# nanoporetech/bonito

Hardware: AMD Instinct MI355X
Metric: signal samples/sec/GPU (chunk=10000, batch=512) + read accuracy vs ref (higher is better)
Workload: dtype f16

## Files before the change

### bonito_amd/csrc/beam.hip

```cpp
#include <stdlib.h>

#include "common.h"
#include "kernels.h"
#include <cstring>
#include "../../include/bh_lse_table.h"

namespace bh {

__device__ const float g_lse_tab[BH_LSE_TABLE_SIZE] = {BH_LSE_TABLE_VALUES};

__device__ __forceinline__ float lse2_tab(float a, float b, const float* tab) {
    float m = fmaxf(a, b);
    float d = fabsf(a - b);
    if (!(d < BH_LSE_RANGE)) return m;
    float x = d * BH_LSE_SCALE;
    int i = (int)x;
    float f = x - (float)i;
    float t0 = tab[i];
    float sp = __fmaf_rn(f, tab[i + 1] - t0, t0);
    return m + sp;
}

__device__ __forceinline__ float lse2_tab_nb(float a, float b, const float* tab) {
    const float m = fmaxf(a, b);
// ... 421 lines not shown
            }
        }
#pragma unroll
        for (int i = 0; i < 3; ++i) selm[i] = __ballot(hi[i] || selb[i]);
    }
    int before = 0;
#pragma unroll
    for (int i = 0; i < 3; ++i) {
        sel[i] = (selm[i] >> lane) & 1ull;
        slot[i] = before + popc64(selm[i] & lanemask_lt(lane));
        before += popc64(selm[i]);
    }
    return before;
}

constexpr int NBK = 256;
constexpr int BKE = 2;
constexpr unsigned TAG_MASK = 0x1ffffu;

struct BeamTable {
    int* cnt;
    uint2_t* ent;
    int* ov_cnt;
    uint2_t* ov;
};

__device__ __forceinline__ unsigned bucket_match(const uint4_t& e0, unsigned hash, unsigned want) {
    unsigned d = 32u;
    d = min(d, e0.x == hash ? e0.y - want : 32u);
    d = min(d, e0.z == hash ? e0.w - want : 32u);
    return d;
}

__device__ __forceinline__ void dma16(const char* g, char* lds) {
    const unsigned l = (unsigned)__builtin_amdgcn_readfirstlane((int)(unsigned)(size_t)(__attribute__((address_space(3))) char*)lds);
    asm volatile("s_mov_b32 m0, %0\n\ts_nop 0\n\tglobal_load_lds_dwordx4 %1, off" ::"s"(l), "v"(g) : "memory");
}
__device__ __forceinline__ void dma16_nt(const char* g, char* lds) {
    const unsigned l = (unsigned)__builtin_amdgcn_readfirstlane((int)(unsigned)(size_t)(__attribute__((address_space(3))) char*)lds);
    asm volatile("s_mov_b32 m0, %0\n\ts_nop 0\n\tglobal_load_lds_dwordx4 %1, off nt" ::"s"(l), "v"(g) : "memory");
}

#include "../../include/bh_bs2.h"
typedef float float2_t __attribute__((ext_vector_type(2)));

__device__ __forceinline__ float2_t fma2(float2_t a, float2_t b, float2_t c) { return __builtin_elementwise_fma(a, b, c); }
__device__ __forceinline__ float2_t splat2(float v) { return float2_t{v, v}; }

__device__ __forceinline__ float2_t bs2_exp2(float2_t x) {
    x.x = __builtin_amdgcn_fmed3f(x.x, -BH_BS2_XMAX, BH_BS2_XMAX);
    x.y = __builtin_amdgcn_fmed3f(x.y, -BH_BS2_XMAX, BH_BS2_XMAX);
    const float2_t t = fma2(x, splat2(BH_BS2_LOG2E), splat2(BH_BS2_MAGIC));
    const float2_t n = t - splat2(BH_BS2_MAGIC);
    const float2_t f = fma2(x, splat2(BH_BS2_LOG2E), -n);
    float2_t p = splat2(BH_BS2_E5);
    p = fma2(p, f, splat2(BH_BS2_E4));
    p = fma2(p, f, splat2(BH_BS2_E3));
    p = fma2(p, f, splat2(BH_BS2_E2));
    p = fma2(p, f, splat2(BH_BS2_E1));
    p = fma2(p, f, splat2(BH_BS2_E0));
    float2_t r;
    r.x = __uint_as_float(__float_as_uint(p.x) + (__float_as_uint(t.x) << 23));
    r.y = __uint_as_float(__float_as_uint(p.y) + (__float_as_uint(t.y) << 23));
    return r;
}
__device__ __forceinline__ float bs2_exp1(float x) { return bs2_exp2(float2_t{x, x}).x; }
// ... 28 lines not shown
        v = fmaxf(v, dpp_f<0x4E, 0xF>(v));
    }
    if constexpr (GL >= 16) {
        v = fmaxf(v, dpp_f<0x124, 0xF>(v));
        v = fmaxf(v, dpp_f<0x128, 0xF>(v));
    }
    if constexpr (GL == 64) {
        v = fmaxf(v, dpp_f<0x142, 0xA>(v));
        v = fmaxf(v, dpp_f<0x143, 0xC>(v));
        v = __builtin_bit_cast(float, __builtin_amdgcn_readlane(__builtin_bit_cast(int, v), 63));
    }
    return v;
}
template <int GL>
__device__ __forceinline__ float group_sum(float v) {
    if constexpr (GL >= 4) {
        v += dpp_f<0xB1, 0xF>(v);
        v += dpp_f<0x4E, 0xF>(v);
    }
    if constexpr (GL >= 16) {
        v += dpp_f<0x124, 0xF>(v);
        v += dpp_f<0x128, 0xF>(v);
    }
    if constexpr (GL == 64) {
        const float r1 = __builtin_bit_cast(float, __builtin_amdgcn_readlane(__builtin_bit_cast(int, v), 15));
        const float r2 = __builtin_bit_cast(float, __builtin_amdgcn_readlane(__builtin_bit_cast(int, v), 31));
        const float r3 = __builtin_bit_cast(float, __builtin_amdgcn_readlane(__builtin_bit_cast(int, v), 47));
        const float r4 = __builtin_bit_cast(float, __builtin_amdgcn_readlane(__builtin_bit_cast(int, v), 63));
        v = (r1 + r2) + (r3 + r4);
    }
    return v;
}

template <int STATE_LEN>
struct Bs2Geo {
    static constexpr int S = 1 << (2 * STATE_LEN), Q = S / 4;
    static constexpr int GL = Q < 64 ? Q : 64;
    static constexpr int CPWV = 64 / GL;
    static constexpr int WPC = Q <= 64 ? 1 : Q / 64;
    static constexpr int UT = WPC * 64;
    static constexpr int UPB = CPWV > 1 ? 1 : 256 / UT;
    static constexpr int CPB = UPB * CPWV;
    static constexpr int ROW = 4 * S * 2;
    static constexpr int PP = CPWV * S / 2;
    static constexpr int UNIT_LDS = 2 * BS2_R * CPWV * ROW + CPWV * 2 * S * 4 + 64;
};

template <int STATE_LEN>
__global__ __launch_bounds__(256) void bs2_backward_kernel(Bs2Args p) {
    using G = Bs2Geo<STATE_LEN>;
    constexpr int S = G::S, Q = G::Q, WPC = G::WPC, GL = G::GL, CPWV = G::CPWV;
    extern __shared__ __attribute__((aligned(16))) char smem[];
    const int T = p.T;
    const int unit = threadIdx.x / G::UT, tu = threadIdx.x - unit * G::UT;
    const int lane = threadIdx.x & 63, wv = tu >> 6;
    const int c = WPC == 1 ? lane / GL : 0;
    const int m = WPC == 1 ? lane - c * GL : tu;
    const int n0 = (blockIdx.x * G::UPB + unit) * CPWV;
    const int n = n0 + c;
    const bool live = n < p.N;
    const int nn = live ? n : p.N - 1;
    char* mine = smem + (size_t)unit * G::UNIT_LDS;
    half_t* rows = (half_t*)mine;
    float* pb = (float*)(mine + 2 * BS2_R * CPWV * G::ROW) + (size_t)c * 2 * S;
    float* mxs = (float*)(mine + 2 * BS2_R * CPWV * G::ROW) + (size_t)CPWV * 2 * S;
    float* bn = p.b + (long)nn * (T + 1) * S;
    const float eb = bs2_exp1(p.blank);

    auto stage = [&](int k) {
        const int u0 = k * BS2_R, nr = min(BS2_R, T - u0);
        for (int r = 0; r < nr; ++r) {
            char* dst = (char*)(rows + (size_t)((k & 1) * BS2_R + r) * CPWV * 4 * S);
            const long trow = (long)(T - 1 - (u0 + r)) * 4 * S;
#pragma unroll
            for (int i0 = 0; i0 < G::PP; i0 += G::UT) {
                const int q = i0 + wv * 64 + lane;
                const int qc = q / (S / 2), qp = q - qc * (S / 2);
                const int qn = min(n0 + qc, p.N - 1);
                const char* src = (const char*)(p.scores + (long)qn * T * 4 * S + trow) + (long)qp * 16;
                if (p.nt) dma16_nt(src, dst + (size_t)(i0 + wv * 64) * 16);
                else dma16(src, dst + (size_t)(i0 + wv * 64) * 16);
            }
        }
    };
#pragma unroll
    for (int l = 0; l < 4; ++l) pb[m + l * Q] = 1.0f;
    if (WPC > 1 && tu < 4) mxs[tu] = 1.0f;
    if (WPC == 1 && live) {
#pragma unroll
        for (int l = 0; l < 4; ++l) bn[(long)T * S + m + l * Q] = 1.0f;
    }
    if (T > 0) stage(0);
    int cur = 0;
    const int nblk = (T + BS2_R - 1) / BS2_R;
    for (int k = 0; k < nblk; ++k) {
        const int u0 = k * BS2_R, nr = min(BS2_R, T - u0);
        asm volatile("s_waitcnt vmcnt(0)" ::: "memory");
        if (WPC > 1) __syncthreads();
        if (k + 1 < nblk) stage(k + 1);
        for (int r = 0; r < nr; ++r) {
            const int t = T - 1 - (u0 + r);
            const float* prev = pb + cur * S;
            const half_t* row = rows + ((size_t)((k & 1) * BS2_R + r) * CPWV + c) * 4 * S;
            const uint4_t w0 = *(const uint4_t*)(row + 16 * m);
            const uint4_t w1 = *(const uint4_t*)(row + 16 * m + 8);
            float4_t succ = *(const float4_t*)(prev + 4 * m);
            float own[4];
#pragma unroll
            for (int l = 0; l < 4; ++l) own[l] = prev[m + l * Q];
            if (WPC > 1) {
                const float4_t mv = *(const float4_t*)(mxs + cur * 4);
                const float mx = fmaxf(fmaxf(mv.x, mv.y), fmaxf(mv.z, mv.w));
                const unsigned eb23 = ((__float_as_uint(mx) >> 23) - 127u) << 23;
#pragma unroll
                for (int l = 0; l < 4; ++l) own[l] = __uint_as_float(__float_as_uint(own[l]) - eb23);
#pragma unroll
                for (int x = 0; x < 4; ++x) succ[x] = __uint_as_float(__float_as_uint(succ[x]) - eb23);
                if (live) {
#pragma unroll
                    for (int l = 0; l < 4; ++l) {
                        if (p.nt) __builtin_nontemporal_store(own[l], bn + (long)(t + 1) * S + m + l * Q);
                        else bn[(long)(t + 1) * S + m + l * Q] = own[l];
                    }
                }
            }
            const unsigned w[8] = {w0.x, w0.y, w0.z, w0.w, w1.x, w1.y, w1.z, w1.w};
            float2_t acc01, acc23;
            acc01 = fma2(splat2(eb), float2_t{own[0], own[1]}, splat2(BH_BS2_TINY));
            acc23 = fma2(splat2(eb), float2_t{own[2], own[3]}, splat2(BH_BS2_TINY));
#pragma unroll
            for (int x = 0; x < 4; ++x) {
                const half2_t h01 = __builtin_bit_cast(half2_t, w[2 * x]), h23 = __builtin_bit_cast(half2_t, w[2 * x + 1]);
                const float2_t e01 = bs2_exp2(float2_t{(float)h01.x, (float)h01.y});
                const float2_t e23 = bs2_exp2(float2_t{(float)h23.x, (float)h23.y});
                acc01 = fma2(e01, splat2(succ[x]), acc01);
                acc23 = fma2(e23, splat2(succ[x]), acc23);
// ... 3 lines not shown
            float* nextb = pb + (cur ^ 1) * S;
            if (WPC > 1) {
                if (lane == 0) mxs[(cur ^ 1) * 4 + wv] = mx;
#pragma unroll
                for (int l = 0; l < 4; ++l) nextb[m + l * Q] = raw[l];
                __syncthreads();
            } else {
                const unsigned eb23 = ((__float_as_uint(mx) >> 23) - 127u) << 23;
#pragma unroll
                for (int l = 0; l < 4; ++l) raw[l] = __uint_as_float(__float_as_uint(raw[l]) - eb23);
#pragma unroll
                for (int l = 0; l < 4; ++l) nextb[m + l * Q] = raw[l];
                if (live) {
#pragma unroll
                    for (int l = 0; l < 4; ++l) {
                        if (p.nt) __builtin_nontemporal_store(raw[l], bn + (long)t * S + m + l * Q);
                        else bn[(long)t * S + m + l * Q] = raw[l];
                    }
                }
            }
            cur ^= 1;
        }
    }
    if (WPC > 1 && live) {
        const float* prev = pb + cur * S;
        const float4_t mv = *(const float4_t*)(mxs + cur * 4);
        const float mx = fmaxf(fmaxf(mv.x, mv.y), fmaxf(mv.z, mv.w));
        const unsigned eb23 = ((__float_as_uint(mx) >> 23) - 127u) << 23;
#pragma unroll
        for (int l = 0; l < 4; ++l) bn[m + l * Q] = __uint_as_float(__float_as_uint(prev[m + l * Q]) - eb23);
    }
}

template <int STATE_LEN>
__host__ __device__ constexpr int beam_wave_lds() {
    constexpr int S = 1 << (2 * STATE_LEN), BTB = beam_btb<STATE_LEN>();
    return 2 * (BTB * 4 * S * 2 + BTB * S * 4) + NBK * BKE * 8 + MAXW * (16 + 8 + 8) + (NBK + 4) * 4 + BTB * MAXW;
}
constexpr int BEAM_TAB_LDS = (BH_LSE_TABLE_SIZE + 2) * 4;

template <int STATE_LEN>
__host__ __device__ constexpr int scan_wave_lds() { return 2 * (1 << (2 * STATE_LEN)) * 4 + 64; }
__device__ __forceinline__ float wave_sum_f32(float v) {
    v += dpp_f<0xB1, 0xF>(v);
    v += dpp_f<0x4E, 0xF>(v);
    v += dpp_f<0x124, 0xF>(v);
    v += dpp_f<0x128, 0xF>(v);
    const float r1 = __builtin_bit_cast(float, __builtin_amdgcn_readlane(__builtin_bit_cast(int, v), 15));
    const float r2 = __builtin_bit_cast(float, __builtin_amdgcn_readlane(__builtin_bit_cast(int, v), 31));
    const float r3 = __builtin_bit_cast(float, __builtin_amdgcn_readlane(__builtin_bit_cast(int, v), 47));
    const float r4 = __builtin_bit_cast(float, __builtin_amdgcn_readlane(__builtin_bit_cast(int, v), 63));
    return (r1 + r2) + (r3 + r4);
}

template <int STATE_LEN>
__device__ __forceinline__ void scan_lin_lane(float ebl, const half_t* row, const float* ap, int m, float (&anew)[4]) {
    constexpr int S = 1 << (2 * STATE_LEN), Q = S / 4;
    const uint4_t w0 = *(const uint4_t*)(row + 16 * m), w1 = *(const uint4_t*)(row + 16 * m + 8);
    const float4_t own = *(const float4_t*)(ap + 4 * m);
    float pr[4];
#pragma unroll
    for (int r = 0; r < 4; ++r) pr[r] = ap[r * Q + m];
    const unsigned w[8] = {w0.x, w0.y, w0.z, w0.w, w1.x, w1.y, w1.z, w1.w};
#pragma unroll
    for (int k = 0; k < 4; ++k) {
        const half2_t cap = {(half_t)BH_BS2_XMAX, (half_t)BH_BS2_XMAX};
        const half2_t h01 = __builtin_elementwise_min(__builtin_bit_cast(half2_t, w[2 * k]), cap);
        const half2_t h23 = __builtin_elementwise_min(__builtin_bit_cast(half2_t, w[2 * k + 1]), cap);
        float a = __fmaf_rn(ebl, own[k], BH_BS2_TINY);
        a = __fmaf_rn(__expf((float)h01.x), pr[0], a);
        a = __fmaf_rn(__expf((float)h01.y), pr[1], a);
        a = __fmaf_rn(__expf((float)h23.x), pr[2], a);
        a = __fmaf_rn(__expf((float)h23.y), pr[3], a);
        anew[k] = a;
    }
}

template <int STATE_LEN>
__device__ __forceinline__ void scan_step(float ebl, const half_t* row, const float* bnext, float* ap, float* an, int m, bool act, float* Pt) {
    constexpr int S = 1 << (2 * STATE_LEN), Q = S / 4, GL = Q < 64 ? Q : 64;
    float anew[4];
    scan_lin_lane<STATE_LEN>(ebl, row, ap, m, anew);
    const float4_t bnext4 = *(const float4_t*)(bnext + 4 * m);
    const float mx = group_max<GL>(fmaxf(fmaxf(anew[0], anew[1]), fmaxf(anew[2], anew[3])));
    const unsigned e23 = ((__float_as_uint(mx) >> 23) - 127u) << 23;
    float4_t o;
#pragma unroll
    for (int k = 0; k < 4; ++k) o[k] = __uint_as_float(__float_as_uint(anew[k]) - e23);
    if (act) *(float4_t*)(an + 4 * m) = o;
    float cls[4];
#pragma unroll
    for (int k = 0; k < 4; ++k) cls[k] = group_sum<GL>(o[k] * bnext4[k]);
    const float inv = 1.0f / ((cls[0] + cls[1]) + (cls[2] + cls[3]));
    if (GL == 1) {
        if (act) *(float4_t*)Pt = float4_t{cls[0] * inv, cls[1] * inv, cls[2] * inv, cls[3] * inv};
    } else if (act && m < 4) {
        Pt[m] = (m == 0 ? cls[0] : m == 1 ? cls[1] : m == 2 ? cls[2] : cls[3]) * inv;
    }
}

struct Bs2FwdArgs {
    const half_t* scores;
    const float* b;
    float* P;
    int N, T;
    float blank;
// ... 132 lines not shown
    char* mine = smem + BEAM_TAB_LDS + wave * beam_wave_lds<STATE_LEN>();
    half_t* st_sc = (half_t*)mine;
    float* st_b = (float*)(st_sc + 2 * BTB * 4 * S);
    constexpr int SCAN_LDS = scan_wave_lds<STATE_LEN>();
    char* scan_mem = smem + BEAM_TAB_LDS + CPW * beam_wave_lds<STATE_LEN>() + wave * SCAN_LDS;
    if (scan_role) {
        float* al = (float*)scan_mem;
        const int sm = QS >= 64 ? lane : lane - (lane / GLS) * GLS;
        if (slot_ok) *(float4_t*)(al + 4 * sm) = float4_t{1.0f, 1.0f, 1.0f, 1.0f};
        const float ebl = __expf(__builtin_amdgcn_fmed3f(p.blank, -BH_BS2_XMAX, BH_BS2_XMAX));
        float* Pn = p.P + (long)n * T * 4;
        int cb = 0;
        for (int tb0 = 0, blk = 0; tb0 < T; tb0 += BTB, ++blk) {
            const int nsteps = min(BTB, T - tb0);
            __syncthreads();
            const half_t* blk_sc = st_sc + (blk & 1) * BTB * 4 * S;
            const float* blk_b = st_b + (blk & 1) * BTB * S;
            for (int u = 0; u < nsteps; ++u) {
                scan_step<STATE_LEN>(ebl, blk_sc + u * 4 * S, blk_b + u * S, al + cb * S, al + (cb ^ 1) * S, sm, slot_ok, Pn + (long)(tb0 + u) * 4);
                cb ^= 1;
            }
        }
        return;
    }
    BeamTable tb;
    tb.ent = (uint2_t*)(st_b + 2 * BTB * S);
    uint4_t* b_elem = (uint4_t*)(tb.ent + NBK * BKE);
    uint2_t* m_pair = (uint2_t*)(b_elem + MAXW);
    tb.ov = m_pair + MAXW;
    tb.cnt = (int*)(tb.ov + MAXW);
    tb.ov_cnt = tb.cnt + NBK;
    int* hist = tb.cnt;
    uint8_t* st_bp = (uint8_t*)(tb.ov_cnt + 4);

    const half_t* sc = p.scores + (long)n * T * 4 * S;
    const float* bn = p.beta + (long)n * (T + 1) * S;
    uint8_t* bpn = p.bp + (long)n * T * MAXW;

    long long dsec[6] = {0, 0, 0, 0, 0, 0};
    const int ce[3] = {lane & (MAXW - 1), lane >> 2, 16 + (lane >> 2)};
    const int mx = lane & 3;
    const bool stay_lane = lane < MAXW;

    int nb;
#pragma unroll
    for (int i = 0; i < NBK * BKE / 64; ++i) tb.ent[lane + 64 * i] = uint2_t{0u, 0xffffffffu};
    if (lane < MAXW) tb.ov[lane] = uint2_t{0u, 0xffffffffu};
    *(uint4_t*)(tb.cnt + 4 * lane) = uint4_t{0u, 0u, 0u, 0u};
    if (lane < 4) tb.ov_cnt[lane] = 0;
    if (lane < MAXW) m_pair[lane] = uint2_t{0u, 0xffffffffu};
    if (lane < MAXW) b_elem[lane] = uint4_t{0u, 0u, 0u, 0u};
    {
        const int per = (S + 63) / 64;
        unsigned prefix = 0u;
        const int want = W < S ? W : S;
        for (int bit = 31; bit >= 0; --bit) {
            const unsigned trial = prefix | (1u << bit);
            int cnt = 0;
            for (int i = 0; i < per; ++i) {
                const int s = i * 64 + lane;
                const unsigned u = s < S ? bs_ukey(bn[s]) : 0u;
                cnt += popc64(__ballot(u >= trial));
            }
            if (cnt >= want) prefix = trial;
        }
        int n_gt = 0;
        for (int i = 0; i < per; ++i) {
            const int s = i * 64 + lane;
            const unsigned u = s < S ? bs_ukey(bn[s]) : 0u;
            n_gt += popc64(__ballot(u > prefix));
        }
        const int need = want - n_gt;
// ... 25 lines not shown
        dma_rows((const char*)(bn + (long)(tb0 + 1) * S), (char*)(st_b + which * BTB * S), nsteps * S / 4);
    };
    if (T > 0) stage(0, 0);
    for (int tb0 = 0, blk = 0; tb0 < T; tb0 += BTB, ++blk) {
        const int nsteps = min(BTB, T - tb0);
        {
            long long ts0 = 0;
            if (DBG) ts0 = __builtin_readcyclecounter();
            asm volatile("s_waitcnt vmcnt(0)" ::: "memory");
            if (FUSE) __syncthreads();
            if (DBG) dsec[5] += __builtin_readcyclecounter() - ts0;
            if (tb0 + BTB < T) stage(tb0 + BTB, (blk + 1) & 1);
        }
        const half_t* blk_sc = st_sc + (blk & 1) * BTB * 4 * S;
        const float* blk_b = st_b + (blk & 1) * BTB * S;
        for (int u = 0; u < nsteps; ++u) {
            const half_t* row = blk_sc + u * 4 * S;
            const float* b1 = blk_b + u * S;
            const unsigned tag = ((unsigned)(tb0 + u) & TAG_MASK) << 15;
            long long tc0 = 0;
            if (DBG) tc0 = __builtin_readcyclecounter();
            float cs[3];
            unsigned ch[3];
            int cst[3], cinfo[3];
            uint4_t el[3];
#pragma unroll
            for (int i = 0; i < 3; ++i) el[i] = b_elem[ce[i]];
            float mv[3], bg[3];
            uint4_t ent0[3];
            {
                const int es = (int)(el[0].x & (unsigned)(S - 1));
                cst[0] = es; ch[0] = el[0].y; cinfo[0] = ce[0];
                bg[0] = b1[es];
                if (stay_lane && ce[0] < nb) {
                    const int bk = (int)(ch[0] & (NBK - 1));
                    const int pos = atomicAdd(&tb.cnt[bk], 1);
                    const uint2_t e{ch[0], tag | ((unsigned)es << 5) | (unsigned)lane};
                    if (pos < BKE) tb.ent[bk * BKE + pos] = e;
                    else tb.ov[atomicAdd(tb.ov_cnt, 1)] = e;
                }
            }
#pragma unroll
            for (int i = 1; i < 3; ++i) {
                const int es = (int)(el[i].x & (unsigned)(S - 1));
                const int s2 = ((es << 2) | mx) & (S - 1);
                cst[i] = s2;
                ch[i] = bs_mix(el[i].y, mx);
                cinfo[i] = ce[i] | (1 << 5) | (mx << 6);
                mv[i] = (float)row[s2 * 4 + (es >> sh)];
                bg[i] = b1[s2];
                ent0[i] = *(const uint4_t*)(tb.ent + (int)(ch[i] & (NBK - 1)) * BKE);
            }
            const int n_ov = tb.ov_cnt[0];
            cs[0] = (stay_lane && ce[0] < nb) ? __uint_as_float(el[0].z) + p.blank : -INFINITY;
            unsigned dhit[3];
#pragma unroll
            for (int i = 1; i < 3; ++i) {
                cs[i] = ce[i] < nb ? __uint_as_float(el[i].z) + mv[i] : -INFINITY;
                dhit[i] = bucket_match(ent0[i], ch[i], tag | ((unsigned)cst[i] << 5));
            }
            if (n_ov > 0) {
                for (int k = 0; k < n_ov; ++k) {
                    const uint2_t e = tb.ov[k];
#pragma unroll
                    for (int i = 1; i < 3; ++i)
                        dhit[i] = min(dhit[i], e.x == ch[i] ? e.y - (tag | ((unsigned)cst[i] << 5)) : 32u);
                }
            }
#pragma unroll
            for (int i = 1; i < 3; ++i)
                if (ce[i] < nb && dhit[i] < 32u) {
                    m_pair[dhit[i]] = uint2_t{__float_as_uint(cs[i]), (unsigned)cinfo[i]};
                    cs[i] = -INFINITY;
                }
            *(uint4_t*)(tb.cnt + 4 * lane) = uint4_t{0u, 0u, 0u, 0u};
            if (lane < 4) tb.ov_cnt[lane] = 0;
            if (DBG) { const long long t1 = __builtin_readcyclecounter(); dsec[0] += t1 - tc0; tc0 = t1; }
            {
                const uint2_t mp = m_pair[ce[0]];
                const bool merged = stay_lane && ce[0] < nb && (int)mp.y >= 0;
                const float ms = __uint_as_float(mp.x);
                const float lse = lse2_tab_nb(cs[0], ms, tab);
                if (merged && ms > cs[0]) cinfo[0] = (int)mp.y;
                if (merged) cs[0] = lse;
            }
            float key[3];
            float best = -INFINITY;
#pragma unroll
            for (int i = 0; i < 3; ++i) {
                key[i] = cs[i] + bs2_log(bg[i]);
                best = fmaxf(best, key[i]);
            }
            best = wave_max_f32(best);
            const float thr = best - p.cut;
            unsigned uk[3];
#pragma unroll
            for (int i = 0; i < 3; ++i) uk[i] = key[i] >= thr ? bs_ukey(key[i]) : 0u;
            if (DBG) { const long long t1 = __builtin_readcyclecounter(); dsec[1] += t1 - tc0; tc0 = t1; }
            bool sel[3];
            int slot[3];
            const int nnew = hist_select(key, uk, W, lane, thr, p.inv_bin, hist, sel, slot, bs_ukey(thr), bs_ukey(best));
            if (DBG) { const long long t1 = __builtin_readcyclecounter(); dsec[2] += t1 - tc0; tc0 = t1; }
            const unsigned ubest = bs_ukey(best);
            float shift = 0.0f;
            {
                int found = 0;
#pragma unroll
                for (int i = 0; i < 3; ++i) {
                    const unsigned long long mm = __ballot(sel[i] && uk[i] == ubest);
                    if (!found && mm) {
                        const int src = __ffsll((long long)mm) - 1;
                        shift = __uint_as_float((unsigned)__builtin_amdgcn_readlane((int)__float_as_uint(cs[i]), src));
                        found = 1;
                    }
                }
            }
#pragma unroll
            for (int i = 0; i < 3; ++i)
                if (sel[i]) {
                    b_elem[slot[i]] = uint4_t{(unsigned)cst[i], ch[i], __float_as_uint(cs[i] - shift), 0u};
                    st_bp[u * MAXW + slot[i]] = (uint8_t)cinfo[i];
                }
            if (lane < MAXW) m_pair[lane] = uint2_t{0u, 0xffffffffu};
            nb = nnew;
            if (DBG) { const long long t1 = __builtin_readcyclecounter(); dsec[3] += t1 - tc0; dsec[4] += nb; }
        }
        for (int i = lane; i < nsteps * MAXW / 4; i += 64)
            ((unsigned*)(bpn + (long)tb0 * MAXW))[i] = ((const unsigned*)st_bp)[i];
    }
    {
        const unsigned u = lane < nb ? bs_ukey(__uint_as_float(b_elem[lane].z)) : 0u;
        unsigned m = u;
#pragma unroll
        for (int off = 32; off > 0; off >>= 1) m = max(m, (unsigned)__shfl_xor((int)m, off));
        const unsigned long long mm = __ballot(u == m && lane < nb);
        if (lane == 0) p.final_slot[n] = __ffsll((long long)mm) - 1;
    }
    if (DBG && lane == 0)
        for (int i = 0; i < 6; ++i) p.dbg[(long)n * 8 + i] = dsec[i];
}

struct FinArgs {
    const uint8_t* bp;
    const int* final_slot;
    const float* P;
    int N, T;
    float q_scale, q_offset;
    int8_t* sequence;
    int8_t* qstring;
    int8_t* moves;
    float* qfloat;
};

constexpr int FTB = 256;

__global__ __launch_bounds__(64) void beam_finalize_kernel(FinArgs p) {
    __shared__ __attribute__((aligned(16))) uint8_t st[FTB * MAXW];
    __shared__ int8_t res_m[FTB], res_s[FTB];
    __shared__ int s_r;
    const int n = blockIdx.x, lane = threadIdx.x;
    const int T = p.T;
    const uint8_t* bp = p.bp + (long)n * T * MAXW;
    const float* P = p.P + (long)n * T * 4;
    int8_t* sq = p.sequence + (long)n * T;
    int8_t* qs = p.qstring + (long)n * T;
    int8_t* mv = p.moves + (long)n * T;
    float* qf = p.qfloat ? p.qfloat + (long)n * T : nullptr;
    if (lane == 0) s_r = p.final_slot[n];
    for (int thi = T; thi > 0; thi -= FTB) {
        const int tlo = max(0, thi - FTB);
        const int nbytes = (thi - tlo) * MAXW;
        const uint4_t* src = (const uint4_t*)(bp + (long)tlo * MAXW);
// ... 104 lines not shown
    using namespace bh;
    BH_REQUIRE(state_len >= 1 && state_len <= 5 && N > 0 && T > 0, "posterior_viterbi: bad shape");
    int S = 1;
    for (int i = 0; i < state_len; ++i) S *= 4;
    auto align = [](size_t x) { return (x + 255) / 256 * 256; };
    char* w = (char*)workspace;
    float* beta = (float*)w;   w += align((size_t)N * (T + 1) * S * sizeof(float));
    double* Bcum = (double*)w; w += align((size_t)N * (T + 1) * sizeof(double));
    double* logZ = (double*)w;
    uint8_t* bp = (uint8_t*)workspace + bh_k_beam_workspace(N, T, state_len);
    ScanArgs sa{(const half_t*)scores, N, T, S, state_len, blank, beta, Bcum, logZ, nullptr, g_decode_nt, 1};
    const int threads = S < 64 ? 64 : S;
    {
        int b_threads = 0;
        size_t b_lds = 0;
        backward_geometry(S, N, sa.cpb, b_threads, b_lds);
        if (b_lds > 64 * 1024) BH_CHECK_HIP(bh_max_lds((const void*)crf_backward_kernel, (int)b_lds));
        hipLaunchKernelGGL(crf_backward_kernel, dim3((N + sa.cpb - 1) / sa.cpb), dim3(b_threads), b_lds, stream, sa);
        sa.cpb = 1;
    }
    PostVitArgs pa{sa, bp, moves, path};
    int TB = (32 * 1024) / S; if (TB > 512) TB = 512; if (TB < 1) TB = 1;
    const size_t lds_pv = (size_t)(BH_LSE_TABLE_SIZE + 2 + 4 * S + 4) * sizeof(float) + (size_t)TB * S + 2 * TB + 32;
    hipLaunchKernelGGL(crf_posterior_viterbi_kernel, dim3(N), dim3(threads), lds_pv, stream, pa);
    BH_CHECK_HIP(hipGetLastError());
    return 0;
}

namespace {
struct SideStream { hipStream_t stream = nullptr; hipEvent_t fork = nullptr, join = nullptr; };
int g_beam_select = 0;
int g_beam_fork = -1;
int g_beam_cpw = 0;
int g_beam_fuse = -1;
SideStream* side_stream(int S) {
    if (g_beam_fork == 0 || (g_beam_fork < 0 && S > 64 && S < 1024)) return nullptr;
    thread_local SideStream per_dev[16];
    int dev = 0;
    if (hipGetDevice(&dev) != hipSuccess || dev < 0 || dev >= 16) return nullptr;
    SideStream& s = per_dev[dev];
    if (!s.stream) {
        if (hipStreamCreateWithFlags(&s.stream, hipStreamNonBlocking) != hipSuccess) { s.stream = nullptr; return nullptr; }
        if (hipEventCreateWithFlags(&s.fork, hipEventDisableTiming) != hipSuccess ||
            hipEventCreateWithFlags(&s.join, hipEventDisableTiming) != hipSuccess) return nullptr;
    }
    return &s;
}
}

int bh_k_beam_search(const void* scores, int N, int T, int state_len, int beam_width, float beam_cut,
                     float blank, float q_scale, float q_offset, void* workspace, int8_t* sequence,
                     int8_t* qstring, int8_t* moves, float* qfloat, hipStream_t stream) {
    using namespace bh;
    BH_REQUIRE(state_len >= 1 && state_len <= 5, "beam_search: state_len must be in 1..5 (got %d)", state_len);
    BH_REQUIRE(N > 0 && T > 0, "beam_search: empty problem N=%d T=%d", N, T);
    BH_REQUIRE(beam_width >= 1 && beam_width <= 32, "beam_search: beam_width must be in 1..32 (got %d)", beam_width);
    BH_REQUIRE(beam_cut >= 1.0f, "beam_search: beam_cut must be >= 1");
    BH_REQUIRE(T < (1 << 17), "beam_search: at most 131071 steps per chunk (got %d)", T);
    int S = 1;
    for (int i = 0; i < state_len; ++i) S *= 4;
    auto align = [](size_t x) { return (x + 255) / 256 * 256; };
    char* w = (char*)workspace;
    float* beta = (float*)w;   w += align((size_t)N * (T + 1) * S * sizeof(float));
    w += align((size_t)N * (T + 1) * sizeof(double));
    w += align((size_t)N * sizeof(double));
    float* P = (float*)w;      w += align((size_t)N * T * 4 * sizeof(float));
    uint8_t* bp = (uint8_t*)w; w += align((size_t)N * T * 32);
    int* fin = (int*)w;         w += align((size_t)N * sizeof(int));
    long long* dbg = getenv("BH_BEAM_DEBUG") ? (long long*)w : nullptr;

    const bool fuse = g_beam_fuse != 0 && S <= 256;
    {
        Bs2Args a2{(const half_t*)scores, beta, N, T, blank, g_decode_nt};
        auto launch_bwd = [&](auto kern, int cpb, size_t lds, int threads) -> int {
            if (lds > 64 * 1024) BH_CHECK_HIP(bh_max_lds((const void*)kern, (int)lds));
            hipLaunchKernelGGL(kern, dim3((N + cpb - 1) / cpb), dim3(threads), lds, stream, a2);
            return 0;
        };
        int rc = -2;
        switch (state_len) {
            case 1: rc = launch_bwd(bs2_backward_kernel<1>, Bs2Geo<1>::CPB, (size_t)Bs2Geo<1>::UPB * Bs2Geo<1>::UNIT_LDS, Bs2Geo<1>::UPB * Bs2Geo<1>::UT); break;
            case 2: rc = launch_bwd(bs2_backward_kernel<2>, Bs2Geo<2>::CPB, (size_t)Bs2Geo<2>::UPB * Bs2Geo<2>::UNIT_LDS, Bs2Geo<2>::UPB * Bs2Geo<2>::UT); break;
            case 3: rc = launch_bwd(bs2_backward_kernel<3>, Bs2Geo<3>::CPB, (size_t)Bs2Geo<3>::UPB * Bs2Geo<3>::UNIT_LDS, Bs2Geo<3>::UPB * Bs2Geo<3>::UT); break;
            case 4: rc = launch_bwd(bs2_backward_kernel<4>, Bs2Geo<4>::CPB, (size_t)Bs2Geo<4>::UPB * Bs2Geo<4>::UNIT_LDS, Bs2Geo<4>::UPB * Bs2Geo<4>::UT); break;
            case 5: rc = launch_bwd(bs2_backward_kernel<5>, Bs2Geo<5>::CPB, (size_t)Bs2Geo<5>::UPB * Bs2Geo<5>::UNIT_LDS, Bs2Geo<5>::UPB * Bs2Geo<5>::UT); break;
        }
        if (rc) return rc;
    }
    SideStream* side = fuse ? nullptr : side_stream(S);
    const bool fork = side != nullptr;
    if (fork) {
        BH_CHECK_HIP(hipEventRecord(side->fork, stream));
        BH_CHECK_HIP(hipStreamWaitEvent(side->stream, side->fork, 0));
    }
    if (!fuse) {
        Bs2FwdArgs f2{(const half_t*)scores, beta, P, N, T, blank, g_decode_nt};
        hipStream_t fs = fork ? side->stream : stream;
        auto launch_fwd = [&](auto kern, int cpb, size_t chunk_lds) -> int {
            const size_t lds = (size_t)cpb * chunk_lds;
            if (lds > 64 * 1024) BH_CHECK_HIP(bh_max_lds((const void*)kern, (int)lds));
            hipLaunchKernelGGL(kern, dim3((N + cpb - 1) / cpb), dim3(256), lds, fs, f2);
            return 0;
        };
        int rc = -2;
        switch (state_len) {
            case 1: rc = launch_fwd(bs2_forward_post_kernel<1>, Bs2FwdGeo<1>::CPB, Bs2FwdGeo<1>::CHUNK_LDS); break;
            case 2: rc = launch_fwd(bs2_forward_post_kernel<2>, Bs2FwdGeo<2>::CPB, Bs2FwdGeo<2>::CHUNK_LDS); break;
            case 3: rc = launch_fwd(bs2_forward_post_kernel<3>, Bs2FwdGeo<3>::CPB, Bs2FwdGeo<3>::CHUNK_LDS); break;
            case 4: rc = launch_fwd(bs2_forward_post_kernel<4>, Bs2FwdGeo<4>::CPB, Bs2FwdGeo<4>::CHUNK_LDS); break;
            case 5: rc = launch_fwd(bs2_forward_post_kernel<5>, Bs2FwdGeo<5>::CPB, Bs2FwdGeo<5>::CHUNK_LDS); break;
        }
        if (rc) return rc;
    }
    if (fork) BH_CHECK_HIP(hipEventRecord(side->join, side->stream));
    BeamArgs ba{(const half_t*)scores, beta, N, T, S, state_len, beam_width, blank, logf(beam_cut), bp, fin, dbg,
                g_beam_select ? 0.0f : 256.0f / fmaxf(logf(beam_cut), 1e-6f), P, g_decode_nt};
    auto launch_beam = [&](auto kern, int cpw, size_t wave_lds, size_t scan_lds = 0) -> int {
        const size_t lds_beam = (size_t)BEAM_TAB_LDS + cpw * (wave_lds + scan_lds);
        if (lds_beam > 64 * 1024)
            BH_CHECK_HIP(bh_max_lds((const void*)kern, (int)lds_beam));
        hipLaunchKernelGGL(kern, dim3((N + cpw - 1) / cpw), dim3(64 * (cpw + (!scan_lds ? 0 : S >= 256 ? cpw : 1))), lds_beam, stream, ba);
        return 0;
    };
    int lrc = -2;
    int cpw4 = g_beam_cpw;
    if (fuse && state_len == 4 && cpw4 <= 0) {
        const long cus = bh_cu_count();
        cpw4 = (long)N <= 5 * cus ? 1 : (long)N <= 6 * cus ? 2 : 4;
    }
    if (false) {
    } else if (fuse && state_len == 4 && !dbg && cpw4 == 4) {
        lrc = launch_beam(beam_kernel<4, 4, false, true>, 4, beam_wave_lds<4>(), scan_wave_lds<4>());
    } else if (fuse && state_len == 4 && !dbg && cpw4 == 2) {
        lrc = launch_beam(beam_kernel<4, 2, false, true>, 2, beam_wave_lds<4>(), scan_wave_lds<4>());
    } else if (fuse) {
        switch (state_len * 2 + (dbg ? 1 : 0)) {
            case 2: lrc = launch_beam(beam_kernel<1, 4, false, true>, 4, beam_wave_lds<1>(), scan_wave_lds<1>()); break;
            case 3: lrc = launch_beam(beam_kernel<1, 4, true, true>, 4, beam_wave_lds<1>(), scan_wave_lds<1>()); break;
            case 4: lrc = launch_beam(beam_kernel<2, 4, false, true>, 4, beam_wave_lds<2>(), scan_wave_lds<2>()); break;
            case 5: lrc = launch_beam(beam_kernel<2, 4, true, true>, 4, beam_wave_lds<2>(), scan_wave_lds<2>()); break;
            case 6: lrc = launch_beam(beam_kernel<3, 4, false, true>, 4, beam_wave_lds<3>(), scan_wave_lds<3>()); break;
            case 7: lrc = launch_beam(beam_kernel<3, 4, true, true>, 4, beam_wave_lds<3>(), scan_wave_lds<3>()); break;
            case 8: lrc = launch_beam(beam_kernel<4, 1, false, true>, 1, beam_wave_lds<4>(), scan_wave_lds<4>()); break;
            case 9: lrc = launch_beam(beam_kernel<4, 1, true, true>, 1, beam_wave_lds<4>(), scan_wave_lds<4>()); break;
        }
    } else
    switch (state_len * 2 + (dbg ? 1 : 0)) {
        case 2: lrc = launch_beam(beam_kernel<1, 4, false>, 4, beam_wave_lds<1>()); break;
        case 3: lrc = launch_beam(beam_kernel<1, 4, true>, 4, beam_wave_lds<1>()); break;
        case 4: lrc = launch_beam(beam_kernel<2, 4, false>, 4, beam_wave_lds<2>()); break;
        case 5: lrc = launch_beam(beam_kernel<2, 4, true>, 4, beam_wave_lds<2>()); break;
        case 6: lrc = launch_beam(beam_kernel<3, 4, false>, 4, beam_wave_lds<3>()); break;
        case 7: lrc = launch_beam(beam_kernel<3, 4, true>, 4, beam_wave_lds<3>()); break;
        case 8: lrc = launch_beam(beam_kernel<4, 1, false>, 1, beam_wave_lds<4>()); break;
        case 9: lrc = launch_beam(beam_kernel<4, 1, true>, 1, beam_wave_lds<4>()); break;
        case 10: lrc = launch_beam(beam_kernel<5, 1, false>, 1, beam_wave_lds<5>()); break;
        case 11: lrc = launch_beam(beam_kernel<5, 1, true>, 1, beam_wave_lds<5>()); break;
    }
    if (lrc) return lrc;
    if (fork) BH_CHECK_HIP(hipStreamWaitEvent(stream, side->join, 0));
    FinArgs fa{bp, fin, P, N, T, q_scale, q_offset, sequence, qstring, moves, qfloat};
    hipLaunchKernelGGL(beam_finalize_kernel, dim3(N), dim3(64), 0, stream, fa);
    BH_CHECK_HIP(hipGetLastError());
    return 0;
}

int bh_k_decode_set_option(const char* name, int value) {
    if (name && !strcmp(name, "beam_fork")) { g_beam_fork = value; return 0; }
    if (name && !strcmp(name, "beam_select")) { g_beam_select = value; return 0; }
    if (name && !strcmp(name, "beam_fuse")) { g_beam_fuse = value; return 0; }
    if (name && !strcmp(name, "beam_cpw")) { g_beam_cpw = value; return 0; }
    if (name && !strcmp(name, "decode_nt")) { g_decode_nt = value; return 0; }
    if (name && !strcmp(name, "viterbi_quad")) { bh::g_viterbi_quad = value; return 0; }
    return 1;
}
```

Baseline: 422.2 million.

## Make beam step branch-free with sink-slot LDS stores and exp2 scan

Replaces divergent conditional LDS writes in the beam step (hash insert, merge pairs, selected-elements and backpointers) with unconditional stores that redirect inactive lanes to a per-lane LDS sink area. The shift computation moves ahead of histogram selection, and m_pair and overflow-count resets are folded into earlier points. The fused scan replaces __expf with a clamped hardware exp2 on scaled input. It also wires DBG variants for state_len 4 and adds a timing bucket. The aim is to cut branch divergence and exec-mask overhead in the serial per-step beam loop, at the cost of extra LDS space and wasted stores. The shift no longer checks sel[i], which could change results if the best key is not selected.

Result: no change. 426.5 million (median of 6 runs) (+1.0%).

```diff
diff --git a/bonito_amd/csrc/beam.hip b/bonito_amd/csrc/beam.hip
--- a/bonito_amd/csrc/beam.hip
+++ b/bonito_amd/csrc/beam.hip
@@ -477,6 +477,13 @@
     return d;
 }
 
+template <class T>
+__device__ __forceinline__ void lds_store_sel(bool c, T* a, T* b, T v) {
+    unsigned x = c ? (unsigned)(size_t)(__attribute__((address_space(3))) T*)a : (unsigned)(size_t)(__attribute__((address_space(3))) T*)b;
+    asm volatile("" : "+v"(x));
+    *(__attribute__((address_space(3))) T*)(size_t)x = v;
+}
+
 __device__ __forceinline__ void dma16(const char* g, char* lds) {
     const unsigned l = (unsigned)__builtin_amdgcn_readfirstlane((int)(unsigned)(size_t)(__attribute__((address_space(3))) char*)lds);
     asm volatile("s_mov_b32 m0, %0\n\ts_nop 0\n\tglobal_load_lds_dwordx4 %1, off" ::"s"(l), "v"(g) : "memory");
@@ -710,10 +717,11 @@
     }
 }
 
+constexpr int BEAM_SINK = 16;
 template <int STATE_LEN>
 __host__ __device__ constexpr int beam_wave_lds() {
     constexpr int S = 1 << (2 * STATE_LEN), BTB = beam_btb<STATE_LEN>();
-    return 2 * (BTB * 4 * S * 2 + BTB * S * 4) + NBK * BKE * 8 + MAXW * (16 + 8 + 8) + (NBK + 4) * 4 + BTB * MAXW;
+    return 2 * (BTB * 4 * S * 2 + BTB * S * 4) + NBK * BKE * 8 + MAXW * (16 + 8 + 8) + (NBK + 4) * 4 + BTB * MAXW + 64 * BEAM_SINK;
 }
 constexpr int BEAM_TAB_LDS = (BH_LSE_TABLE_SIZE + 2) * 4;
 
@@ -731,6 +739,11 @@
     return (r1 + r2) + (r3 + r4);
 }
 
+constexpr float SCAN_LOG2E = 1.44269504088896340736f;
+constexpr float SCAN_CAP2 = BH_BS2_XMAX * SCAN_LOG2E;
+__device__ __forceinline__ float scan_exp(half_t h) {
+    return __builtin_amdgcn_exp2f(fminf(__builtin_fmaf((float)h, SCAN_LOG2E, 0.0f), SCAN_CAP2));
+}
 template <int STATE_LEN>
 __device__ __forceinline__ void scan_lin_lane(float ebl, const half_t* row, const float* ap, int m, float (&anew)[4]) {
     constexpr int S = 1 << (2 * STATE_LEN), Q = S / 4;
@@ -742,14 +755,12 @@
     const unsigned w[8] = {w0.x, w0.y, w0.z, w0.w, w1.x, w1.y, w1.z, w1.w};
 #pragma unroll
     for (int k = 0; k < 4; ++k) {
-        const half2_t cap = {(half_t)BH_BS2_XMAX, (half_t)BH_BS2_XMAX};
-        const half2_t h01 = __builtin_elementwise_min(__builtin_bit_cast(half2_t, w[2 * k]), cap);
-        const half2_t h23 = __builtin_elementwise_min(__builtin_bit_cast(half2_t, w[2 * k + 1]), cap);
+        const half2_t h01 = __builtin_bit_cast(half2_t, w[2 * k]), h23 = __builtin_bit_cast(half2_t, w[2 * k + 1]);
         float a = __fmaf_rn(ebl, own[k], BH_BS2_TINY);
-        a = __fmaf_rn(__expf((float)h01.x), pr[0], a);
-        a = __fmaf_rn(__expf((float)h01.y), pr[1], a);
-        a = __fmaf_rn(__expf((float)h23.x), pr[2], a);
-        a = __fmaf_rn(__expf((float)h23.y), pr[3], a);
+        a = __fmaf_rn(scan_exp(h01.x), pr[0], a);
+        a = __fmaf_rn(scan_exp(h01.y), pr[1], a);
+        a = __fmaf_rn(scan_exp(h23.x), pr[2], a);
+        a = __fmaf_rn(scan_exp(h23.y), pr[3], a);
         anew[k] = a;
     }
 }
@@ -948,12 +959,13 @@
     tb.ov_cnt = tb.cnt + NBK;
     int* hist = tb.cnt;
     uint8_t* st_bp = (uint8_t*)(tb.ov_cnt + 4);
+    char* my_sink = (char*)(st_bp + BTB * MAXW) + BEAM_SINK * lane;
 
     const half_t* sc = p.scores + (long)n * T * 4 * S;
     const float* bn = p.beta + (long)n * (T + 1) * S;
     uint8_t* bpn = p.bp + (long)n * T * MAXW;
 
-    long long dsec[6] = {0, 0, 0, 0, 0, 0};
+    long long dsec[7] = {0, 0, 0, 0, 0, 0, 0};
     const int ce[3] = {lane & (MAXW - 1), lane >> 2, 16 + (lane >> 2)};
     const int mx = lane & 3;
     const bool stay_lane = lane < MAXW;
@@ -1045,12 +1057,14 @@
                 const int es = (int)(el[0].x & (unsigned)(S - 1));
                 cst[0] = es; ch[0] = el[0].y; cinfo[0] = ce[0];
                 bg[0] = b1[es];
-                if (stay_lane && ce[0] < nb) {
-                    const int bk = (int)(ch[0] & (NBK - 1));
-                    const int pos = atomicAdd(&tb.cnt[bk], 1);
-                    const uint2_t e{ch[0], tag | ((unsigned)es << 5) | (unsigned)lane};
-                    if (pos < BKE) tb.ent[bk * BKE + pos] = e;
-                    else tb.ov[atomicAdd(tb.ov_cnt, 1)] = e;
+                const bool ins = stay_lane && ce[0] < nb;
+                const int bk = (int)(ch[0] & (NBK - 1));
+                const int pos = atomicAdd(&tb.cnt[ins ? bk : lane], ins ? 1 : 0);
+                const uint2_t e{ch[0], tag | ((unsigned)es << 5) | (unsigned)lane};
+                lds_store_sel(ins && pos < BKE, tb.ent + bk * BKE + pos, (uint2_t*)my_sink, e);
+                const bool ovf = ins && pos >= BKE;
+                if (__ballot(ovf)) {
+                    if (ovf) tb.ov[atomicAdd(tb.ov_cnt, 1)] = e;
                 }
             }
 #pragma unroll
@@ -1068,10 +1082,10 @@
             cs[0] = (stay_lane && ce[0] < nb) ? __uint_as_float(el[0].z) + p.blank : -INFINITY;
             unsigned dhit[3];
 #pragma unroll
-            for (int i = 1; i < 3; ++i) {
-                cs[i] = ce[i] < nb ? __uint_as_float(el[i].z) + mv[i] : -INFINITY;
-                dhit[i] = bucket_match(ent0[i], ch[i], tag | ((unsigned)cst[i] << 5));
-            }
+            for (int i = 1; i < 3; ++i) dhit[i] = bucket_match(ent0[i], ch[i], tag | ((unsigned)cst[i] << 5));
+            asm volatile("" : "+v"(mv[1]), "+v"(mv[2]));
+#pragma unroll
+            for (int i = 1; i < 3; ++i) cs[i] = ce[i] < nb ? __uint_as_float(el[i].z) + mv[i] : -INFINITY;
             if (n_ov > 0) {
                 for (int k = 0; k < n_ov; ++k) {
                     const uint2_t e = tb.ov[k];
@@ -1079,24 +1093,26 @@
                     for (int i = 1; i < 3; ++i)
                         dhit[i] = min(dhit[i], e.x == ch[i] ? e.y - (tag | ((unsigned)cst[i] << 5)) : 32u);
                 }
-            }
-#pragma unroll
-            for (int i = 1; i < 3; ++i)
-                if (ce[i] < nb && dhit[i] < 32u) {
-                    m_pair[dhit[i]] = uint2_t{__float_as_uint(cs[i]), (unsigned)cinfo[i]};
-                    cs[i] = -INFINITY;
-                }
+                tb.ov_cnt[0] = 0;
+            }
+#pragma unroll
+            for (int i = 1; i < 3; ++i) {
+                const bool hit = ce[i] < nb && dhit[i] < 32u;
+                lds_store_sel(hit, m_pair + dhit[i], (uint2_t*)my_sink, uint2_t{__float_as_uint(cs[i]), (unsigned)cinfo[i]});
+                cs[i] = hit ? -INFINITY : cs[i];
+            }
             *(uint4_t*)(tb.cnt + 4 * lane) = uint4_t{0u, 0u, 0u, 0u};
-            if (lane < 4) tb.ov_cnt[lane] = 0;
             if (DBG) { const long long t1 = __builtin_readcyclecounter(); dsec[0] += t1 - tc0; tc0 = t1; }
             {
                 const uint2_t mp = m_pair[ce[0]];
+                m_pair[ce[0]] = uint2_t{0u, 0xffffffffu};
                 const bool merged = stay_lane && ce[0] < nb && (int)mp.y >= 0;
                 const float ms = __uint_as_float(mp.x);
                 const float lse = lse2_tab_nb(cs[0], ms, tab);
                 if (merged && ms > cs[0]) cinfo[0] = (int)mp.y;
                 if (merged) cs[0] = lse;
             }
+            if (DBG) { const long long t1 = __builtin_readcyclecounter(); dsec[1] += t1 - tc0; tc0 = t1; }
             float key[3];
             float best = -INFINITY;
 #pragma unroll
@@ -1109,32 +1125,25 @@
             unsigned uk[3];
 #pragma unroll
             for (int i = 0; i < 3; ++i) uk[i] = key[i] >= thr ? bs_ukey(key[i]) : 0u;
-            if (DBG) { const long long t1 = __builtin_readcyclecounter(); dsec[1] += t1 - tc0; tc0 = t1; }
+            const unsigned ubest = bs_ukey(best);
+            float shift;
+            {
+                const unsigned long long m0 = __ballot(uk[0] == ubest), m1 = __ballot(uk[1] == ubest), m2 = __ballot(uk[2] == ubest);
+                const unsigned long long mm = m0 ? m0 : m1 ? m1 : m2;
+                const float c = m0 ? cs[0] : m1 ? cs[1] : cs[2];
+                const int src = mm ? __ffsll((long long)mm) - 1 : 0;
+                shift = mm ? __uint_as_float((unsigned)__builtin_amdgcn_readlane((int)__float_as_uint(c), src)) : 0.0f;
+            }
+            if (DBG) { const long long t1 = __builtin_readcyclecounter(); dsec[6] += t1 - tc0; tc0 = t1; }
             bool sel[3];
             int slot[3];
             const int nnew = hist_select(key, uk, W, lane, thr, p.inv_bin, hist, sel, slot, bs_ukey(thr), bs_ukey(best));
             if (DBG) { const long long t1 = __builtin_readcyclecounter(); dsec[2] += t1 - tc0; tc0 = t1; }
-            const unsigned ubest = bs_ukey(best);
-            float shift = 0.0f;
-            {
-                int found = 0;
-#pragma unroll
-                for (int i = 0; i < 3; ++i) {
-                    const unsigned long long mm = __ballot(sel[i] && uk[i] == ubest);
-                    if (!found && mm) {
-                        const int src = __ffsll((long long)mm) - 1;
-                        shift = __uint_as_float((unsigned)__builtin_amdgcn_readlane((int)__float_as_uint(cs[i]), src));
-                        found = 1;
-                    }
-                }
-            }
-#pragma unroll
-            for (int i = 0; i < 3; ++i)
-                if (sel[i]) {
-                    b_elem[slot[i]] = uint4_t{(unsigned)cst[i], ch[i], __float_as_uint(cs[i] - shift), 0u};
-                    st_bp[u * MAXW + slot[i]] = (uint8_t)cinfo[i];
-                }
-            if (lane < MAXW) m_pair[lane] = uint2_t{0u, 0xffffffffu};
+#pragma unroll
+            for (int i = 0; i < 3; ++i) {
+                lds_store_sel(sel[i], b_elem + slot[i], (uint4_t*)my_sink, uint4_t{(unsigned)cst[i], ch[i], __float_as_uint(cs[i] - shift), 0u});
+                lds_store_sel(sel[i], st_bp + u * MAXW + slot[i], (uint8_t*)my_sink, (uint8_t)cinfo[i]);
+            }
             nb = nnew;
             if (DBG) { const long long t1 = __builtin_readcyclecounter(); dsec[3] += t1 - tc0; dsec[4] += nb; }
         }
@@ -1150,7 +1159,7 @@
         if (lane == 0) p.final_slot[n] = __ffsll((long long)mm) - 1;
     }
     if (DBG && lane == 0)
-        for (int i = 0; i < 6; ++i) p.dbg[(long)n * 8 + i] = dsec[i];
+        for (int i = 0; i < 7; ++i) p.dbg[(long)n * 8 + i] = dsec[i];
 }
 
 struct FinArgs {
@@ -1418,10 +1427,12 @@
         cpw4 = (long)N <= 5 * cus ? 1 : (long)N <= 6 * cus ? 2 : 4;
     }
     if (false) {
-    } else if (fuse && state_len == 4 && !dbg && cpw4 == 4) {
-        lrc = launch_beam(beam_kernel<4, 4, false, true>, 4, beam_wave_lds<4>(), scan_wave_lds<4>());
-    } else if (fuse && state_len == 4 && !dbg && cpw4 == 2) {
-        lrc = launch_beam(beam_kernel<4, 2, false, true>, 2, beam_wave_lds<4>(), scan_wave_lds<4>());
+    } else if (fuse && state_len == 4 && cpw4 == 4) {
+        lrc = dbg ? launch_beam(beam_kernel<4, 4, true, true>, 4, beam_wave_lds<4>(), scan_wave_lds<4>())
+                  : launch_beam(beam_kernel<4, 4, false, true>, 4, beam_wave_lds<4>(), scan_wave_lds<4>());
+    } else if (fuse && state_len == 4 && cpw4 == 2) {
+        lrc = dbg ? launch_beam(beam_kernel<4, 2, true, true>, 2, beam_wave_lds<4>(), scan_wave_lds<4>())
+                  : launch_beam(beam_kernel<4, 2, false, true>, 2, beam_wave_lds<4>(), scan_wave_lds<4>());
     } else if (fuse) {
         switch (state_len * 2 + (dbg ? 1 : 0)) {
             case 2: lrc = launch_beam(beam_kernel<1, 4, false, true>, 4, beam_wave_lds<1>(), scan_wave_lds<1>()); break;
```

## Software-pipeline exp computation in single-wave backward kernel and make row count tunable

Applied to the files above, without the earlier changes.

Templates the backward beam-scoring kernel on the number of staged rows per block and adds a dedicated path for the single-wave-per-chunk case. That path computes the exponentiated transition weights for the next timestep while the current step's accumulation and normalisation run, so exp latency overlaps the serial recurrence. It also adds a runtime option to pick 1 or 2 staged rows for state_len 4. The cost is extra registers for the prefetched exps and more kernel instantiations.

Measured after the change: 419.1 million before, 418.9 million after (median of 3 runs). No clear change (-0.0%).

```diff
diff --git a/bonito_amd/csrc/beam.hip b/bonito_amd/csrc/beam.hip
--- a/bonito_amd/csrc/beam.hip
+++ b/bonito_amd/csrc/beam.hip
@@ -571,7 +571,7 @@
     return v;
 }
 
-template <int STATE_LEN>
+template <int STATE_LEN, int R = BS2_R>
 struct Bs2Geo {
     static constexpr int S = 1 << (2 * STATE_LEN), Q = S / 4;
     static constexpr int GL = Q < 64 ? Q : 64;
@@ -582,12 +582,12 @@
     static constexpr int CPB = UPB * CPWV;
     static constexpr int ROW = 4 * S * 2;
     static constexpr int PP = CPWV * S / 2;
-    static constexpr int UNIT_LDS = 2 * BS2_R * CPWV * ROW + CPWV * 2 * S * 4 + 64;
+    static constexpr int UNIT_LDS = 2 * R * CPWV * ROW + CPWV * 2 * S * 4 + 64;
 };
 
-template <int STATE_LEN>
+template <int STATE_LEN, int R>
 __global__ __launch_bounds__(256) void bs2_backward_kernel(Bs2Args p) {
-    using G = Bs2Geo<STATE_LEN>;
+    using G = Bs2Geo<STATE_LEN, R>;
     constexpr int S = G::S, Q = G::Q, WPC = G::WPC, GL = G::GL, CPWV = G::CPWV;
     extern __shared__ __attribute__((aligned(16))) char smem[];
     const int T = p.T;
@@ -601,15 +601,15 @@
     const int nn = live ? n : p.N - 1;
     char* mine = smem + (size_t)unit * G::UNIT_LDS;
     half_t* rows = (half_t*)mine;
-    float* pb = (float*)(mine + 2 * BS2_R * CPWV * G::ROW) + (size_t)c * 2 * S;
-    float* mxs = (float*)(mine + 2 * BS2_R * CPWV * G::ROW) + (size_t)CPWV * 2 * S;
+    float* pb = (float*)(mine + 2 * R * CPWV * G::ROW) + (size_t)c * 2 * S;
+    float* mxs = (float*)(mine + 2 * R * CPWV * G::ROW) + (size_t)CPWV * 2 * S;
     float* bn = p.b + (long)nn * (T + 1) * S;
     const float eb = bs2_exp1(p.blank);
 
     auto stage = [&](int k) {
-        const int u0 = k * BS2_R, nr = min(BS2_R, T - u0);
+        const int u0 = k * R, nr = min(R, T - u0);
         for (int r = 0; r < nr; ++r) {
-            char* dst = (char*)(rows + (size_t)((k & 1) * BS2_R + r) * CPWV * 4 * S);
+            char* dst = (char*)(rows + (size_t)((k & 1) * R + r) * CPWV * 4 * S);
             const long trow = (long)(T - 1 - (u0 + r)) * 4 * S;
 #pragma unroll
             for (int i0 = 0; i0 < G::PP; i0 += G::UT) {
@@ -629,18 +629,79 @@
 #pragma unroll
         for (int l = 0; l < 4; ++l) bn[(long)T * S + m + l * Q] = 1.0f;
     }
+    int cur = 0;
+    const int nblk = (T + R - 1) / R;
+    if constexpr (WPC == 1) {
+        float2_t e01[4], e23[4];
+        auto exps = [&](int u) {
+            const int k = u / R, r = u - k * R;
+            const half_t* row = rows + ((size_t)((k & 1) * R + r) * CPWV + c) * 4 * S;
+            const uint4_t w0 = *(const uint4_t*)(row + 16 * m);
+            const uint4_t w1 = *(const uint4_t*)(row + 16 * m + 8);
+            const unsigned w[8] = {w0.x, w0.y, w0.z, w0.w, w1.x, w1.y, w1.z, w1.w};
+#pragma unroll
+            for (int x = 0; x < 4; ++x) {
+                const half2_t h01 = __builtin_bit_cast(half2_t, w[2 * x]), h23 = __builtin_bit_cast(half2_t, w[2 * x + 1]);
+                e01[x] = bs2_exp2(float2_t{(float)h01.x, (float)h01.y});
+                e23[x] = bs2_exp2(float2_t{(float)h23.x, (float)h23.y});
+            }
+        };
+        if (T > 0) {
+            stage(0);
+            asm volatile("s_waitcnt vmcnt(0)" ::: "memory");
+            if (nblk > 1) stage(1);
+            exps(0);
+        }
+        for (int u = 0; u < T; ++u) {
+            const int t = T - 1 - u;
+            if ((u + 1) % R == 0 && u + 1 < T) {
+                const int k1 = (u + 1) / R;
+                asm volatile("s_waitcnt vmcnt(0)" ::: "memory");
+                if (k1 + 1 < nblk) stage(k1 + 1);
+            }
+            const float* prev = pb + cur * S;
+            const float4_t succ = *(const float4_t*)(prev + 4 * m);
+            float own[4];
+#pragma unroll
+            for (int l = 0; l < 4; ++l) own[l] = prev[m + l * Q];
+            float2_t acc01, acc23;
+            acc01 = fma2(splat2(eb), float2_t{own[0], own[1]}, splat2(BH_BS2_TINY));
+            acc23 = fma2(splat2(eb), float2_t{own[2], own[3]}, splat2(BH_BS2_TINY));
+#pragma unroll
+            for (int x = 0; x < 4; ++x) {
+                acc01 = fma2(e01[x], splat2(succ[x]), acc01);
+                acc23 = fma2(e23[x], splat2(succ[x]), acc23);
+            }
+            exps(u + 1 < T ? u + 1 : u);
+            float raw[4] = {acc01.x, acc01.y, acc23.x, acc23.y};
+            const float mx = group_max<GL>(fmaxf(fmaxf(raw[0], raw[1]), fmaxf(raw[2], raw[3])));
+            const unsigned eb23 = ((__float_as_uint(mx) >> 23) - 127u) << 23;
+#pragma unroll
+            for (int l = 0; l < 4; ++l) raw[l] = __uint_as_float(__float_as_uint(raw[l]) - eb23);
+            float* nextb = pb + (cur ^ 1) * S;
+#pragma unroll
+            for (int l = 0; l < 4; ++l) nextb[m + l * Q] = raw[l];
+            if (live) {
+#pragma unroll
+                for (int l = 0; l < 4; ++l) {
+                    if (p.nt) __builtin_nontemporal_store(raw[l], bn + (long)t * S + m + l * Q);
+                    else bn[(long)t * S + m + l * Q] = raw[l];
+                }
+            }
+            cur ^= 1;
+        }
+        return;
+    }
     if (T > 0) stage(0);
-    int cur = 0;
-    const int nblk = (T + BS2_R - 1) / BS2_R;
     for (int k = 0; k < nblk; ++k) {
-        const int u0 = k * BS2_R, nr = min(BS2_R, T - u0);
+        const int u0 = k * R, nr = min(R, T - u0);
         asm volatile("s_waitcnt vmcnt(0)" ::: "memory");
         if (WPC > 1) __syncthreads();
         if (k + 1 < nblk) stage(k + 1);
         for (int r = 0; r < nr; ++r) {
             const int t = T - 1 - (u0 + r);
             const float* prev = pb + cur * S;
-            const half_t* row = rows + ((size_t)((k & 1) * BS2_R + r) * CPWV + c) * 4 * S;
+            const half_t* row = rows + ((size_t)((k & 1) * R + r) * CPWV + c) * 4 * S;
             const uint4_t w0 = *(const uint4_t*)(row + 16 * m);
             const uint4_t w1 = *(const uint4_t*)(row + 16 * m + 8);
             float4_t succ = *(const float4_t*)(prev + 4 * m);
@@ -1321,6 +1382,7 @@
 int g_beam_select = 0;
 int g_beam_fork = -1;
 int g_beam_cpw = 0;
+int g_bs2_rows = 0;
 int g_beam_fuse = -1;
 SideStream* side_stream(int S) {
     if (g_beam_fork == 0 || (g_beam_fork < 0 && S > 64 && S < 1024)) return nullptr;
@@ -1368,11 +1430,14 @@
         };
         int rc = -2;
         switch (state_len) {
-            case 1: rc = launch_bwd(bs2_backward_kernel<1>, Bs2Geo<1>::CPB, (size_t)Bs2Geo<1>::UPB * Bs2Geo<1>::UNIT_LDS, Bs2Geo<1>::UPB * Bs2Geo<1>::UT); break;
-            case 2: rc = launch_bwd(bs2_backward_kernel<2>, Bs2Geo<2>::CPB, (size_t)Bs2Geo<2>::UPB * Bs2Geo<2>::UNIT_LDS, Bs2Geo<2>::UPB * Bs2Geo<2>::UT); break;
-            case 3: rc = launch_bwd(bs2_backward_kernel<3>, Bs2Geo<3>::CPB, (size_t)Bs2Geo<3>::UPB * Bs2Geo<3>::UNIT_LDS, Bs2Geo<3>::UPB * Bs2Geo<3>::UT); break;
-            case 4: rc = launch_bwd(bs2_backward_kernel<4>, Bs2Geo<4>::CPB, (size_t)Bs2Geo<4>::UPB * Bs2Geo<4>::UNIT_LDS, Bs2Geo<4>::UPB * Bs2Geo<4>::UT); break;
-            case 5: rc = launch_bwd(bs2_backward_kernel<5>, Bs2Geo<5>::CPB, (size_t)Bs2Geo<5>::UPB * Bs2Geo<5>::UNIT_LDS, Bs2Geo<5>::UPB * Bs2Geo<5>::UT); break;
+#define BH_BS2_LAUNCH(SL, RR) launch_bwd(bs2_backward_kernel<SL, RR>, Bs2Geo<SL, RR>::CPB, (size_t)Bs2Geo<SL, RR>::UPB * Bs2Geo<SL, RR>::UNIT_LDS, \
+                                         Bs2Geo<SL, RR>::UPB * Bs2Geo<SL, RR>::UT)
+            case 1: rc = BH_BS2_LAUNCH(1, BS2_R); break;
+            case 2: rc = BH_BS2_LAUNCH(2, BS2_R); break;
+            case 3: rc = BH_BS2_LAUNCH(3, BS2_R); break;
+            case 4: rc = g_bs2_rows == 1 ? BH_BS2_LAUNCH(4, 1) : g_bs2_rows == 2 ? BH_BS2_LAUNCH(4, 2) : BH_BS2_LAUNCH(4, BS2_R); break;
+            case 5: rc = BH_BS2_LAUNCH(5, BS2_R); break;
+#undef BH_BS2_LAUNCH
         }
         if (rc) return rc;
     }
@@ -1459,6 +1524,7 @@
     if (name && !strcmp(name, "beam_select")) { g_beam_select = value; return 0; }
     if (name && !strcmp(name, "beam_fuse")) { g_beam_fuse = value; return 0; }
     if (name && !strcmp(name, "beam_cpw")) { g_beam_cpw = value; return 0; }
+    if (name && !strcmp(name, "bs2_rows")) { g_bs2_rows = value; return 0; }
     if (name && !strcmp(name, "decode_nt")) { g_decode_nt = value; return 0; }
     if (name && !strcmp(name, "viterbi_quad")) { bh::g_viterbi_quad = value; return 0; }
     return 1;
```
